# imatge-upc/rsis

Hardware: AMD Instinct MI355X
Metric: training images/sec at 256x256, T=10, batch=32 per GPU (higher is better)
Workload: dtype f32

## Files before the change

rsis_amd/csrc/api.hip:

```cpp
#include "common.h"
#include "../../include/rsis_hip.h"
#include "launchers.h"
#include <stdlib.h>

static inline int krows_of(int C, int ks) { return rsis_roundup(C * ks * ks, RSIS_KPAD); }
static inline int log2i(int s) { int l = 0; while ((1 << l) < s) ++l; return l; }
static inline bool use_direct(int ks, int stride, int pad) { return ks == 3 && stride == 1 && pad == 1; }
static inline bool use_direct_s2(int ks, int stride, int pad) { return ks == 3 && stride == 2 && pad == 1; }
static inline bool use_direct_f2(int ks, int stride, int pad) {
  static const bool on = !(getenv("RSIS_CONV_F2") && getenv("RSIS_CONV_F2")[0] == '0');
  return on && use_direct_s2(ks, stride, pad);
}
static inline bool use_direct_fwd(int ks, int stride, int pad) { return use_direct(ks, stride, pad) || use_direct_f2(ks, stride, pad); }
static inline int seg_chunks(int nseg, const int* Cseg, int ck) {
  int q = 0;
  for (int s = 0; s < nseg; ++s) q += (Cseg[s] + ck - 1) / ck;
  return q;
}
static inline int direct_rows(int nseg, const int* Cseg) { return seg_chunks(nseg, Cseg, RSIS_CK) * RSIS_CK * 9; }
static inline bool bf16_geom(int ks, int stride, int pad, int Cout) {
  return Cout > 1 && ((ks == 3 && stride == 1 && pad == 1) || (ks == 1 && pad == 0));
}
static inline bool use_bf16(int dtype, int ks, int stride, int pad, int Cout) {
  return dtype == RSIS_DTYPE_BF16 && bf16_geom(ks, stride, pad, Cout);
// ... 348 lines not shown
    a.Ho = Hy; a.Wo = Wy; a.oH = Hx; a.oW = Wx;
    return rsis_launch_conv3x3_direct(a, 2, direct_variant(tile), (hipStream_t)stream);
  }
  if (ks == 1 && pad == 0 && stride > 1) {
    if (!inplace && zero_dsts(a, (hipStream_t)stream)) return RSIS_ERR_LAUNCH;
    a.Ho = Hy; a.Wo = Wy; a.stride = 1; a.sshift = 0; a.ostride = stride;
    return rsis_launch_conv_igemm(a, ks, false, 0, tile, (hipStream_t)stream);
  }
  return rsis_launch_conv_igemm(a, ks, true, 0, tile, (hipStream_t)stream);
}

static int wgrad_route(WgradArgs& a, int ks, int lstm_hid, int dtype) {
  if (dtype == RSIS_DTYPE_BF16_BLK) {
    a.blk = 1;
    return rsis_wgrad_bf16_supported(a, ks) ? 1 : -1;
  }
  if (use_direct(ks, a.stride, a.pad) && a.Cout == 1 && lstm_hid == 0 && rsis_c1_supported(a.Cs) && a.H == a.Ho && a.W == a.Wo && a.W % 4 == 0)
    return 0;
  if (dtype == RSIS_DTYPE_BF16 && rsis_wgrad_bf16_supported(a, ks)) return 1;
  static const bool tiled_ok = !(getenv("RSIS_WGRAD_TILED") && getenv("RSIS_WGRAD_TILED")[0] == '0');
  if (tiled_ok && rsis_wgrad_tiled_supported(a, ks)) return 2;
  return 3;
}
static int wgrad_fill(WgradArgs& a, const float* dy, const float* x, float* dW, int B, int Cs, int H, int W, int Cout, int Ho, int Wo,
                      int ks, int stride, int pad, int Ctot, int c_off, int lstm_hid) {
  if (!dy || !x || !dW || c_off < 0 || c_off + Cs > Ctot) return RSIS_ERR_ARG;
  a = WgradArgs{};
  a.dy = dy; a.x = x; a.dw = dW; a.B = B; a.Cs = Cs; a.H = H; a.W = W; a.Ho = Ho; a.Wo = Wo; a.Cout = Cout;
  a.stride = stride; a.pad = pad; a.ldo = Ctot * ks * ks; a.n_off = c_off * ks * ks; a.interleave_hid = lstm_hid;
  return RSIS_OK;
// ... 623 lines not shown
```

rsis_amd/csrc/common.h:

```cpp
#pragma once
#include <hip/hip_runtime.h>
#include <stdint.h>

#define RSIS_OK 0
#define RSIS_ERR_ARG 1
#define RSIS_ERR_LAUNCH 2
#define RSIS_ERR_UNSUPPORTED 3

#define RSIS_KPAD 32
#define RSIS_CK 8
#define RSIS_CKB3 16
#define RSIS_CKB1 64
#define RSIS_LDW_ALIGN 128
#define RSIS_MAX_SRC 3

enum PackMode {
  PACK_IGEMM_FWD = 0,
  PACK_IGEMM_DGRAD = 1,
  PACK_DIRECT_FWD = 2,
  PACK_DIRECT_DGRAD = 3,
  PACK_DIRECT_DGRAD_S2 = 4,
  PACK_BF16_FWD = 5,
  PACK_BF16_DGRAD = 6,
  PACK_WINO_FWD = 7,
// ... 129 lines not shown
    }
  }
}

struct WgradArgs {
  const float* dy;
  const float* x;
  float* dw;
  int B, Cs, H, W, Ho, Wo, Cout;
  int stride, pad;
  int ldo, n_off;
  int interleave_hid;
  int chunk;
  int n_co_tiles, n_n_tiles;
  int blk;
};

struct BlkConvJob {
  const void* src[RSIS_MAX_SRC];
  int C[RSIS_MAX_SRC];
  int nsrc;
  int B, H, W;
  const void* wp;
  int ldw;
  int Cout;
  const float* bias;
  const void* addend;
  void* dst[2];
  int Cd[2];
  int ndst;
// ... 27 lines not shown
```

rsis_amd/csrc/conv_wgrad_bf16.hip:

```cpp
#include "common.h"
#include "launchers.h"

typedef __attribute__((address_space(3))) void* lds_vp_t;
typedef __bf16 bf16x8 __attribute__((ext_vector_type(8)));
typedef __bf16 bf16x2 __attribute__((ext_vector_type(2)));
typedef float f32x2 __attribute__((ext_vector_type(2)));
typedef unsigned u32x4 __attribute__((ext_vector_type(4)));
#define RSIS_OOB 0x7FFFFFF0u

struct WgradBf16Args {
  const float* dy;
  const float* x;
  float* dw;
  int B, Cs, H, W, Cout;
  int ldo, n_off;
  short interleave_hid;
  short blk;
  int n_co_tiles, n_n_tiles, n_sp_tiles, tiles_per_split;
};

__device__ __forceinline__ unsigned wg_pack2(float lo, float hi) {
  const f32x2 f = {lo, hi};
  return __builtin_bit_cast(unsigned, __builtin_convertvector(f, bf16x2));
}
// ... 10 lines not shown
      v[0] = a[0]; v[1] = a[1]; v[2] = a[2]; v[3] = a[3]; v[4] = b[0]; v[5] = b[1]; v[6] = b[2]; v[7] = b[3];
    } else {
#pragma unroll
      for (int i = 0; i < 8; ++i) {
        const bool ok = ok_row && (unsigned)(gx + i) < (unsigned)W;
        v[i] = __builtin_bit_cast(float, __builtin_amdgcn_raw_buffer_load_b32(r, ok ? (unsigned)(off_elems + i) * 4u : RSIS_OOB, 0, 0));
      }
    }
  }
  __device__ __forceinline__ u32x4 cell() const {
    u32x4 c;
#pragma unroll
    for (int k = 0; k < 4; ++k) c[k] = wg_pack2(v[2 * k], v[2 * k + 1]);
    return c;
  }
};

template <int BM, int TW, int IN>
__device__ __forceinline__ void wgrad3_bf16_body(const WgradBf16Args& p, const int bx, const int by) {
#if __HIP_DEVICE_COMPILE__
  constexpr int TP = 64, TH = TP / TW, GPR = TW / 8, NG = TP / 8, KSTEPS = NG / 2;
  constexpr int WGM = BM / 32, KSPW = 4 / WGM, NGG = KSTEPS / KSPW;
  constexpr int PH = TH + 2, XG = GPR + 2, PWP = XG * 8;
  constexpr int ARS = (TP + 8) * 2;
  constexpr int CHSB = (PH * PWP * 2 + 31) / 32 * 32 + 16;
  constexpr int A_BYTES = BM * ARS, X_BYTES = 32 * CHSB, ST_BYTES = A_BYTES + X_BYTES;
  constexpr int NTA = BM * NG / 256;
  constexpr int XT = 32 * PH * XG, NTX = (XT + 255) / 256;
  constexpr int RED_BYTES = 4 * 8 * 288 * 4;
  static_assert(WGM * KSPW == 4 && KSTEPS % KSPW == 0 && (BM * NG) % 256 == 0, "config");
  constexpr int LDS_BYTES = 2 * ST_BYTES > RED_BYTES ? 2 * ST_BYTES : RED_BYTES;
  __shared__ __attribute__((aligned(16))) char lds[LDS_BYTES];

  const int tid = threadIdx.x, lane = tid & 63, l31 = lane & 31, hi = lane >> 5;
  const int wave = __builtin_amdgcn_readfirstlane(tid >> 6);
  const int wm = wave % WGM, wk = wave / WGM;
  const int H = p.H, W = p.W, HW = H * W, Cs = p.Cs, Cout = p.Cout;
  const int co_t = bx % p.n_co_tiles, n_t = bx / p.n_co_tiles;
  const int co0 = co_t * BM, ci0 = n_t * 32;
  const int tiles_x = (W + TW - 1) / TW, tiles_y = (H + TH - 1) / TH;
  const int t_begin = by * p.tiles_per_split;
  const int t_end = min(t_begin + p.tiles_per_split, p.n_sp_tiles);
  if (t_begin >= t_end) return;

  int a_off[NTA], a_y[NTA], a_x[NTA], a_lds[NTA];
#pragma unroll
  for (int i = 0; i < NTA; ++i) {
    const int e = tid + i * 256;
    const int row = e / NG, G = e % NG;
    a_y[i] = G / GPR; a_x[i] = (G % GPR) * 8;
    a_off[i] = co0 + row < Cout ? row * HW + a_y[i] * W + a_x[i] : -1;
    a_lds[i] = row * ARS + G * 16;
  }
  int x_off[NTX], x_y[NTX], x_x[NTX], x_lds[NTX];
#pragma unroll
  for (int i = 0; i < NTX; ++i) {
    const int e = tid + i * 256;
    const int cl = e / (PH * XG), rem = e - cl * (PH * XG);
    const int py = rem / XG, xg = rem - py * XG;
    x_y[i] = py - 1; x_x[i] = (xg - 1) * 8;
    x_off[i] = (e < XT && ci0 + cl < Cs) ? cl * HW + x_y[i] * W + x_x[i] : (int)0x40000000;
    x_lds[i] = cl * CHSB + (py * PWP + xg * 8) * 2;
  }

  const int a_base = (wm * 32 + l31) * ARS + hi * 16;
  int bo[NGG];
#pragma unroll
  for (int gg = 0; gg < NGG; ++gg) {
    const int G = 2 * (gg * KSPW + wk) + hi;
    bo[gg] = l31 * CHSB + ((G / GPR) * PWP + (G % GPR) * 8 + 8) * 2;
  }

  f32x16 acc[9];
#pragma unroll
  for (int t = 0; t < 9; ++t)
#pragma unroll
    for (int r = 0; r < 16; ++r) acc[t][r] = 0.f;

  int tb = t_begin / (tiles_x * tiles_y);
  int trem = t_begin - tb * (tiles_x * tiles_y);
  int ty = trem / tiles_x, tx = trem - ty * tiles_x;

  Task8<IN == 1> ra[NTA], rxp[NTX];
#define W3_LOAD()                                                                                                  \
  {                                                                                                                \
    const int y0 = ty * TH, x0 = tx * TW;                                                                          \
    const float* ab = p.dy + ((size_t)tb * Cout + co0) * HW;                                                       \
    const __amdgpu_buffer_rsrc_t ra_ = __builtin_amdgcn_make_buffer_rsrc((void*)ab, 0, (Cout - co0) * HW * 4, 0x00020000); \
    const int tsc = y0 * W + x0;                                                                                   \
    _Pragma("unroll") for (int i = 0; i < NTA; ++i)                                                                \
      ra[i].load(ra_, a_off[i] + tsc, a_off[i] >= 0 && y0 + a_y[i] < H, x0 + a_x[i], W);                           \
    const float* xb = p.x + ((size_t)tb * Cs + ci0) * HW;                                                          \
    const __amdgpu_buffer_rsrc_t rx_ = __builtin_amdgcn_make_buffer_rsrc((void*)xb, 0, (Cs - ci0) * HW * 4, 0x00020000); \
    _Pragma("unroll") for (int i = 0; i < NTX; ++i)                                                                \
      rxp[i].load(rx_, x_off[i] + tsc, x_off[i] < 0x20000000 && (unsigned)(y0 + x_y[i]) < (unsigned)H, x0 + x_x[i], W); \
    if (++tx == tiles_x) { tx = 0; if (++ty == tiles_y) { ty = 0; ++tb; } }                                        \
  }
#define W3_STORE(BUF)                                                                                              \
  {                                                                                                                \
    char* st = lds + (BUF) * ST_BYTES;                                                                             \
    _Pragma("unroll") for (int i = 0; i < NTA; ++i) *(u32x4*)(st + a_lds[i]) = ra[i].cell();                       \
    _Pragma("unroll") for (int i = 0; i < NTX; ++i)                                                                \
      if (XT % 256 == 0 || tid + i * 256 < XT) *(u32x4*)(st + A_BYTES + x_lds[i]) = rxp[i].cell();                 \
  }

  W3_LOAD() W3_STORE(0)
  __syncthreads();
  const int ntl = t_end - t_begin;
  for (int t = 0; t < ntl; ++t) {
    const int cur = t & 1;
    if (t + 1 < ntl) W3_LOAD()
    {
      const char* As = lds + cur * ST_BYTES + a_base;
      const char* Xs = lds + cur * ST_BYTES + A_BYTES;
#pragma unroll
      for (int gg = 0; gg < NGG; ++gg) {
        const bf16x8 a = __builtin_bit_cast(bf16x8, *(const u32x4*)(As + (gg * KSPW + wk) * 32));
#pragma unroll
        for (int r = 0; r < 3; ++r) {
          const char* row = Xs + bo[gg] + r * PWP * 2;
          const unsigned d0 = *(const unsigned*)(row - 4);
          const u32x4 m = *(const u32x4*)row;
          const unsigned d5 = *(const unsigned*)(row + 16);
          const u32x4 w0 = {__builtin_amdgcn_alignbit(m[0], d0, 16), __builtin_amdgcn_alignbit(m[1], m[0], 16),
                            __builtin_amdgcn_alignbit(m[2], m[1], 16), __builtin_amdgcn_alignbit(m[3], m[2], 16)};
          const u32x4 w2 = {__builtin_amdgcn_alignbit(m[1], m[0], 16), __builtin_amdgcn_alignbit(m[2], m[1], 16),
                            __builtin_amdgcn_alignbit(m[3], m[2], 16), __builtin_amdgcn_alignbit(d5, m[3], 16)};
          acc[r * 3 + 0] = __builtin_amdgcn_mfma_f32_32x32x16_bf16(a, __builtin_bit_cast(bf16x8, w0), acc[r * 3 + 0], 0, 0, 0);
          acc[r * 3 + 1] = __builtin_amdgcn_mfma_f32_32x32x16_bf16(a, __builtin_bit_cast(bf16x8, m), acc[r * 3 + 1], 0, 0, 0);
          acc[r * 3 + 2] = __builtin_amdgcn_mfma_f32_32x32x16_bf16(a, __builtin_bit_cast(bf16x8, w2), acc[r * 3 + 2], 0, 0, 0);
        }
      }
    }
    if (t + 1 < ntl) W3_STORE(cur ^ 1)
    __syncthreads();
  }
#undef W3_LOAD
#undef W3_STORE

  float* red = (float*)lds + wm * (8 * 288);
  const int nvalid = min(32, Cs - ci0) * 9;
#pragma unroll
  for (int q = 0; q < 4; ++q) {
#pragma unroll
    for (int k = 0; k < KSPW; ++k) {
      if (wk == k) {
#pragma unroll
        for (int t = 0; t < 9; ++t)
#pragma unroll
          for (int r = 0; r < 4; ++r) {
            float* d = red + (r + 4 * hi) * 288 + l31 * 9 + t;
            if (k == 0) *d = acc[t][4 * q + r];
            else *d += acc[t][4 * q + r];
// ... 356 lines not shown
#ifndef W3T_TH_64_32
#define W3T_TH_64_32 4
#define W3T_NR_64_32 2
#endif
#ifndef W3T_TH_64_16
#define W3T_TH_64_16 8
#define W3T_NR_64_16 2
#endif
constexpr int w3t_th(int bm, int tw) {
  return tw == 32 ? (bm == 128 ? 2 : (bm == 64 ? W3T_TH_64_32 : W3T_TH_32_32)) : (tw == 16 ? (bm == 128 ? 4 : (bm == 64 ? W3T_TH_64_16 : 8)) : 8);
}
constexpr int w3t_nr(int bm, int tw) {
  return tw == 32 ? (bm == 128 ? 2 : (bm == 64 ? W3T_NR_64_32 : W3T_NR_32_32)) : (tw == 16 ? (bm == 32 ? 3 : (bm == 64 ? W3T_NR_64_16 : 2)) : (bm == 128 ? 2 : 3));
}

template <int BM, int BN, int WGM, int WGN, int TW, int IN>
__device__ __forceinline__ void wgrad1_bf16_body(const WgradBf16Args& p, const int bx, const int by) {
#if __HIP_DEVICE_COMPILE__
  constexpr int TP = 64, TH = TP / TW, GPR = TW / 8, NG = TP / 8, KSTEPS = NG / 2;
  constexpr int TM = BM / WGM / 32, TN = BN / WGN / 32;
  constexpr int ARS = (TP + 8) * 2;
  constexpr int A_BYTES = BM * ARS, B_BYTES = BN * ARS, ST_BYTES = A_BYTES + B_BYTES;
  constexpr int NTA = BM * NG / 256, NTB = BN * NG / 256;
  static_assert(WGM * WGN == 4 && (BM * NG) % 256 == 0 && (BN * NG) % 256 == 0, "config");
  __shared__ __attribute__((aligned(16))) char lds[2 * ST_BYTES];

  const int tid = threadIdx.x, lane = tid & 63, l31 = lane & 31, hi = lane >> 5;
  const int wave = __builtin_amdgcn_readfirstlane(tid >> 6);
  const int wm = wave / WGN, wn = wave % WGN;
  const int H = p.H, W = p.W, HW = H * W, Cs = p.Cs, Cout = p.Cout;
  const int co_t = bx % p.n_co_tiles, n_t = bx / p.n_co_tiles;
  const int co0 = co_t * BM, n0 = n_t * BN;
  const int tiles_x = (W + TW - 1) / TW, tiles_y = (H + TH - 1) / TH;
  const int t_begin = by * p.tiles_per_split;
  const int t_end = min(t_begin + p.tiles_per_split, p.n_sp_tiles);
  if (t_begin >= t_end) return;

  int a_off[NTA], a_y[NTA], a_x[NTA], a_lds[NTA];
#pragma unroll
  for (int i = 0; i < NTA; ++i) {
// ... 14 lines not shown
  }
  const int a_base = (wm * TM * 32 + l31) * ARS + hi * 16;
  const int b_base = (wn * TN * 32 + l31) * ARS + hi * 16;

  f32x16 acc[TM][TN];
#pragma unroll
  for (int i = 0; i < TM; ++i)
#pragma unroll
    for (int j = 0; j < TN; ++j)
#pragma unroll
      for (int r = 0; r < 16; ++r) acc[i][j][r] = 0.f;

  int tb = t_begin / (tiles_x * tiles_y);
  int trem = t_begin - tb * (tiles_x * tiles_y);
  int ty = trem / tiles_x, tx = trem - ty * tiles_x;

  Task8<IN == 1> ra[NTA], rb[NTB];
#define W1_LOAD()                                                                                                  \
  {                                                                                                                \
    const int y0 = ty * TH, x0 = tx * TW;                                                                          \
    const int tsc = y0 * W + x0;                                                                                   \
    const float* ab = p.dy + ((size_t)tb * Cout + co0) * HW;                                                       \
    const __amdgpu_buffer_rsrc_t ra_ = __builtin_amdgcn_make_buffer_rsrc((void*)ab, 0, (Cout - co0) * HW * 4, 0x00020000); \
    _Pragma("unroll") for (int i = 0; i < NTA; ++i)                                                                \
      ra[i].load(ra_, a_off[i] + tsc, a_off[i] >= 0 && y0 + a_y[i] < H, x0 + a_x[i], W);                           \
    const float* xb = p.x + ((size_t)tb * Cs + n0) * HW;                                                           \
    const __amdgpu_buffer_rsrc_t rb_ = __builtin_amdgcn_make_buffer_rsrc((void*)xb, 0, (Cs - n0) * HW * 4, 0x00020000); \
    _Pragma("unroll") for (int i = 0; i < NTB; ++i)                                                                \
      rb[i].load(rb_, b_off[i] + tsc, b_off[i] >= 0 && y0 + b_y[i] < H, x0 + b_x[i], W);                           \
    if (++tx == tiles_x) { tx = 0; if (++ty == tiles_y) { ty = 0; ++tb; } }                                        \
  }
#define W1_STORE(BUF)                                                                                              \
  {                                                                                                                \
    char* st = lds + (BUF) * ST_BYTES;                                                                             \
    _Pragma("unroll") for (int i = 0; i < NTA; ++i) *(u32x4*)(st + a_lds[i]) = ra[i].cell();                       \
    _Pragma("unroll") for (int i = 0; i < NTB; ++i) *(u32x4*)(st + A_BYTES + b_lds[i]) = rb[i].cell();             \
  }

  W1_LOAD() W1_STORE(0)
  __syncthreads();
  const int ntl = t_end - t_begin;
  for (int t = 0; t < ntl; ++t) {
    const int cur = t & 1;
    if (t + 1 < ntl) W1_LOAD()
    {
      const char* As = lds + cur * ST_BYTES + a_base;
      const char* Bs = lds + cur * ST_BYTES + A_BYTES + b_base;
#pragma unroll
      for (int g = 0; g < KSTEPS; ++g) {
        bf16x8 a[TM], b[TN];
#pragma unroll
        for (int i = 0; i < TM; ++i) a[i] = __builtin_bit_cast(bf16x8, *(const u32x4*)(As + i * 32 * ARS + g * 32));
#pragma unroll
        for (int j = 0; j < TN; ++j) b[j] = __builtin_bit_cast(bf16x8, *(const u32x4*)(Bs + j * 32 * ARS + g * 32));
#pragma unroll
        for (int i = 0; i < TM; ++i)
#pragma unroll
          for (int j = 0; j < TN; ++j) acc[i][j] = __builtin_amdgcn_mfma_f32_32x32x16_bf16(a[i], b[j], acc[i][j], 0, 0, 0);
      }
    }
    if (t + 1 < ntl) W1_STORE(cur ^ 1)
    __syncthreads();
  }
#undef W1_LOAD
#undef W1_STORE

  const __amdgpu_buffer_rsrc_t rdw = __builtin_amdgcn_make_buffer_rsrc((void*)p.dw, 0, (unsigned)((size_t)Cout * p.ldo * 4), 0x00020000);
  const int ihid = p.interleave_hid;
  const unsigned ldb = (unsigned)p.ldo * 4u;
#pragma unroll
  for (int j = 0; j < TN; ++j) {
    const int n = n0 + wn * TN * 32 + j * 32 + l31;
    if (n >= Cs) continue;
#pragma unroll
    for (int i = 0; i < TM; ++i) {
      const int row0 = co0 + wm * TM * 32 + i * 32 + 4 * hi;
      const int rows_left = Cout - row0;
      const unsigned vo = (unsigned)((ihid > 0 ? row0 >> 2 : row0) * p.ldo + p.n_off + n) * 4u;
#pragma unroll
      for (int r = 0; r < 16; ++r) {
// ... 61 lines not shown
  wgrad1_tr_body<BM, BN, TP, NR>(g.job[j], tile, split);
}
template <int BM, int BN, int TP, int NR>
static void w1t_launch_group(const WgradBf16Group& g, int blocks, hipStream_t st) {
  constexpr int lds = w1t_lds_bytes<BM, BN, TP, NR>();
  static const hipError_t once = hipFuncSetAttribute((const void*)wgrad1_tr_group_kernel<BM, BN, TP, NR>, hipFuncAttributeMaxDynamicSharedMemorySize, lds);
  (void)once;
  hipLaunchKernelGGL((wgrad1_tr_group_kernel<BM, BN, TP, NR>), dim3(blocks), dim3(256), lds, st, g);
}
template <int BM, int BN, int WGM, int WGN, int TW, int IN>
__global__ __launch_bounds__(256) void wgrad1_bf16_group_kernel(const WgradBf16Group g) {
  int j, tile, split;
  if (!wgb_find(g, j, tile, split)) return;
  wgrad1_bf16_body<BM, BN, WGM, WGN, TW, IN>(g.job[j], tile, split);
}

static void split_plan(WgradBf16Args& a, int TW, int TH, int ntile, int slots) {
  a.n_sp_tiles = a.B * rsis_cdiv(a.H, TH) * rsis_cdiv(a.W, TW);
  int nsplit = ntile >= slots ? 1 : slots / ntile;
  if (nsplit > 256) nsplit = 256;
  if (nsplit > a.n_sp_tiles / 2) nsplit = a.n_sp_tiles / 2;
  if (nsplit < 1 || rsis_deterministic()) nsplit = 1;
  a.tiles_per_split = rsis_cdiv(a.n_sp_tiles, nsplit);
}

bool rsis_wgrad_bf16_supported(const WgradArgs& w, int ks) {
  if (!(ks == 1 || ks == 3) || w.stride != 1 || w.pad != ks / 2 || w.H != w.Ho || w.W != w.Wo) return false;
  if (w.Cout == 1) return false;
  if (w.blk && ((w.Cout & 7) || (w.Cs & 7))) return false;
  const long img = (long)w.H * w.W * 4;
  return (long)w.Cout * img < (1L << 30) && (long)w.Cs * img < (1L << 30);
}

struct WgbKey { int ks, bm, bn, tw, v4, th; };
static WgbKey wgb_key(const WgradBf16Args& a, int ks) {
  WgbKey k = {ks, 0, 0, 0, 0, 0};
  if (ks == 3) {
    k.tw = a.W > 16 ? 32 : (a.W > 8 ? 16 : 8);
    k.bm = a.Cout <= 32 ? 32 : ((a.Cout <= 64 || a.Cs <= 512) ? 64 : 128);
    k.bn = 32;
  } else {
    k.tw = a.blk ? W1T_TP : 64;
    k.bm = a.Cout <= 64 ? 64 : 128;
    k.bn = a.Cs <= 64 ? 64 : 128;
  }
  k.v4 = a.blk ? 2 : (a.W % 4 == 0 ? 1 : 0);
  k.th = ks == 3 ? (a.blk ? w3t_th(k.bm, k.tw) : 64 / k.tw) : (a.blk ? 1 : 64 / k.tw);
  return k;
}
static inline bool wgb_same(const WgbKey& a, const WgbKey& b) { return a.ks == b.ks && a.bm == b.bm && a.bn == b.bn && a.tw == b.tw && a.v4 == b.v4; }

template <typename LaunchFn>
static int wgb_launch_bucket(WgradBf16Args* jobs, int n, const WgbKey& k, bool alone, LaunchFn launch) {
  const int TH = k.th;
  long total = 0;
  for (int j = 0; j < n; ++j) {
    WgradBf16Args& a = jobs[j];
    a.n_co_tiles = rsis_cdiv(a.Cout, k.bm);
    a.n_n_tiles = rsis_cdiv(a.Cs, k.bn);
    a.n_sp_tiles = a.B * rsis_cdiv(a.H, TH) * rsis_cdiv(a.W, k.tw);
    total += (long)a.n_co_tiles * a.n_n_tiles * a.n_sp_tiles;
  }
  if (alone) {
    WgradBf16Group g = {};
    const int ntile = jobs[0].n_co_tiles * jobs[0].n_n_tiles;
// ... 47 lines not shown
      g.lane_split0[best][e] = (unsigned short)items[i].split;
      blocks[best] += items[i].blocks;
      load[best] += items[i].work;
    }
    int maxb = 0;
    for (int x = 0; x < 8; ++x) { g.lane_start[x][g.lane_n[x]] = blocks[x]; if (blocks[x] > maxb) maxb = blocks[x]; }
    launch(g, 8 * maxb);
    if (rsis_check_launch() != RSIS_OK) return RSIS_ERR_LAUNCH;
    j0 += nj;
  }
  return RSIS_OK;
}

#define WGB3(BMv, TWv)                                                                                             \
  if (k.bm == BMv && k.tw == TWv) {                                                                                \
    if (k.v4 == 2) return wgb_launch_bucket(jobs, n, k, alone, [&](const WgradBf16Group& g, int blocks) {                 \
      w3t_launch_group<BMv, TWv, w3t_th(BMv, TWv), w3t_nr(BMv, TWv)>(g, blocks, st); });                           \
    if (k.v4 == 1) return wgb_launch_bucket(jobs, n, k, alone, [&](const WgradBf16Group& g, int blocks) {                 \
      hipLaunchKernelGGL((wgrad3_bf16_group_kernel<BMv, TWv, 1>), dim3(blocks), dim3(256), 0, st, g); });          \
    return wgb_launch_bucket(jobs, n, k, alone, [&](const WgradBf16Group& g, int blocks) {                                \
      hipLaunchKernelGGL((wgrad3_bf16_group_kernel<BMv, TWv, 0>), dim3(blocks), dim3(256), 0, st, g); });          \
  }
#define WGB1(BMv, BNv)                                                                                             \
  if (k.bm == BMv && k.bn == BNv) {                                                                                \
    if (k.v4 == 2) return wgb_launch_bucket(jobs, n, k, alone, [&](const WgradBf16Group& g, int blocks) {                 \
      w1t_launch_group<BMv, BNv, W1T_TP, w1t_nr(BMv, BNv)>(g, blocks, st); });                                     \
    if (k.v4 == 1) return wgb_launch_bucket(jobs, n, k, alone, [&](const WgradBf16Group& g, int blocks) {                 \
      hipLaunchKernelGGL((wgrad1_bf16_group_kernel<BMv, BNv, 2, 2, 64, 1>), dim3(blocks), dim3(256), 0, st, g); });      \
    return wgb_launch_bucket(jobs, n, k, alone, [&](const WgradBf16Group& g, int blocks) {                                \
      hipLaunchKernelGGL((wgrad1_bf16_group_kernel<BMv, BNv, 2, 2, 64, 0>), dim3(blocks), dim3(256), 0, st, g); });      \
  }
static int wgb_dispatch(WgradBf16Args* jobs, int n, const WgbKey& k, bool alone, hipStream_t st) {
  if (k.ks == 3) {
    WGB3(32, 32) WGB3(64, 32) WGB3(128, 32) WGB3(32, 16) WGB3(64, 16) WGB3(128, 16) WGB3(32, 8) WGB3(64, 8) WGB3(128, 8)
  } else {
    WGB1(64, 64) WGB1(64, 128) WGB1(128, 64) WGB1(128, 128)
  }
  return RSIS_ERR_ARG;
}
#undef WGB3
#undef WGB1

static int wgb_launch_jobs(const WgradArgs* w, int n, int ks, bool alone, hipStream_t st) {
  if (n < 1) return RSIS_OK;
  WgradBf16Args* all = (WgradBf16Args*)malloc(sizeof(WgradBf16Args) * n * 2);
  WgbKey* key = (WgbKey*)malloc(sizeof(WgbKey) * n);
  if (!all || !key) { free(all); free(key); return RSIS_ERR_LAUNCH; }
  WgradBf16Args* bucket = all + n;
  for (int j = 0; j < n; ++j) {
    WgradBf16Args a = {};
    a.dy = w[j].dy; a.x = w[j].x; a.dw = w[j].dw; a.B = w[j].B; a.Cs = w[j].Cs; a.H = w[j].H; a.W = w[j].W; a.Cout = w[j].Cout;
    a.ldo = w[j].ldo; a.n_off = w[j].n_off; a.interleave_hid = (short)w[j].interleave_hid; a.blk = (short)w[j].blk;
    if (ks == 1) { a.W = w[j].H * w[j].W; a.H = 1; }
    all[j] = a;
    key[j] = wgb_key(a, ks);
  }
  int rc = RSIS_OK;
  for (int j = 0; j < n && rc == RSIS_OK; ++j) {
    if (key[j].ks < 0) continue;
    const WgbKey k = key[j];
    int m = 0;
    for (int i = j; i < n; ++i)
      if (key[i].ks >= 0 && wgb_same(key[i], k)) { bucket[m++] = all[i]; key[i].ks = -1; }
    rc = wgb_dispatch(bucket, m, k, alone, st);
  }
  free(all); free(key);
  return rc;
}

int rsis_launch_conv_wgrad_bf16_group(const WgradArgs* w, int n, int ks, hipStream_t st) { return wgb_launch_jobs(w, n, ks, false, st); }
// ... 2 lines not shown
```

rsis_amd/csrc/launchers.h:

```cpp
#pragma once
#include "common.h"
#include "../../include/rsis_hip.h"

int rsis_launch_conv_igemm(ConvArgs& a, int ks, bool dgrad, int epi, int force_tile, hipStream_t st);
int rsis_launch_conv3x3_direct(ConvArgs& a, int epi, int force_variant, hipStream_t st);
int rsis_launch_convlstm_direct_group(ConvArgs* jobs, int n, const int* force_variant, hipStream_t st);
int rsis_launch_conv3x3_direct_group_plain(ConvArgs* jobs, int n, const int* force_variant, hipStream_t st);
int rsis_launch_conv_wino(const float* x, const void* U, const float* bias, const float* addend, float* y, int B, int C, int Cout, int H, int W, hipStream_t st,
                          int precise);
int rsis_launch_conv_wino_group(int n, const float* const* x, const void* const* U, float* const* y, float* const* y1, const int* B, const int* C, const int* Cout,
                                const int* C0, const int* H, const int* W, hipStream_t st);
int rsis_launch_conv_bf16(ConvArgs& a, int ks, int epi, int force_variant, hipStream_t st);
int rsis_launch_conv_blk(ConvArgs& a, int ks, int variant, hipStream_t st);
int rsis_l_blk_from_nchw(const float* x, void* y, int B, int C, int HW, hipStream_t st);
int rsis_l_blk_to_nchw(const void* x, float* y, int B, int C, int HW, hipStream_t st);
int rsis_launch_conv_blk_dec(BlkConvJob* jobs, int n, int epi, const int* force_variant, hipStream_t st);
int rsis_launch_conv_wgrad(WgradArgs& a, int ks, hipStream_t st);
bool rsis_wgrad_bf16_supported(const WgradArgs& w, int ks);
int rsis_launch_conv_wgrad_bf16_group(const WgradArgs* w, int n, int ks, hipStream_t st);
int rsis_launch_conv_wgrad_bf16(const WgradArgs& w, int ks, hipStream_t st);
int rsis_launch_conv_wgrad_tiled_group(const WgradArgs* w, int n, int ks, hipStream_t st);
int rsis_launch_conv_wgrad_tiled(const WgradArgs& w, int ks, hipStream_t st);
bool rsis_wgrad_tiled_supported(const WgradArgs& w, int ks);
bool rsis_c1_supported(int Cin);
int rsis_l_c1_fwd(const float* x, const float* wp, int ldw, const float* bias, float* y, int B, int Cin, int H, int W, int seqT, hipStream_t st);
int rsis_l_c1_dgrad(const float* dy, const float* wd, int ldw, float* dx, int B, int Cin, int H, int W, int seqT, hipStream_t st);
int rsis_l_c1_wgrad(const float* dy, const float* x, float* dw, float* db, int B, int Cin, int H, int W, int seqT, hipStream_t st);
bool rsis_upconv_supported(int C, int Hs, int Ws, int Ho, int Wo);
int rsis_upconv_bwd_blocks(int T, int B, int Hs, int Ws);
int rsis_l_upconv_fwd(const void* h, int h_blk, const float* w, const float* bias, float* out, int T, int B, int Hs, int Ws, int Ho, int Wo, hipStream_t st);
int rsis_l_upconv_bwd(const float* dout, const void* h, int h_blk, const float* w, void* dh, float* dW, float* db, const float* dside, const int* arg,
                      float* partial, int T, int B, int Hs, int Ws, int Ho, int Wo, hipStream_t st);
int rsis_l_pack_batch(const rsis_pack_job* jobs, int njobs, int total_blocks, hipStream_t st);
// ... 88 lines not shown
```

rsis_amd/csrc/limb_split.h:

```cpp
#pragma once

#if defined(__HIPCC__) || defined(__CUDACC__)
#define RSIS_LIMB_HD __host__ __device__
#else
#define RSIS_LIMB_HD
#endif

RSIS_LIMB_HD inline float rsis_limb_hi16(const float v) {
  unsigned u;
  __builtin_memcpy(&u, &v, 4);
  u &= 0xFFFF0000u;
  float r;
  __builtin_memcpy(&r, &u, 4);
  return r;
}

RSIS_LIMB_HD inline void rsis_limb_split3(const float v, float& l0, float& l1, float& l2) {
  l0 = rsis_limb_hi16(v);
  const float r1 = v - l0;
  l1 = rsis_limb_hi16(r1);
  l2 = r1 - l1;
}
```

Before: 963.8.

## Route f32 weight-gradient convs through bf16 MFMA with three-limb split

Adds a path that splits each f32 operand into three bf16 limbs while staging into LDS and computes the weight gradient with six bf16 MFMA products per step, approximating f32 accuracy on matrix cores. By default it is enabled only for selected 3x3 shape classes (tile width 32, in both the small-Cout and large-Cout groups) when not in deterministic mode, and env vars can force it on for all supported shapes or turn it off. The limb kernels use dynamic LDS sized for three planes with a single buffer, so they lose the double-buffered overlap. The large-tile variant also keeps a second set of accumulators that it flushes after every tile, which adds register pressure.

```diff
diff --git a/rsis_amd/csrc/api.hip b/rsis_amd/csrc/api.hip
--- a/rsis_amd/csrc/api.hip
+++ b/rsis_amd/csrc/api.hip
@@ -386,6 +386,11 @@
   if (dtype == RSIS_DTYPE_BF16_BLK) {
     a.blk = 1;
     return rsis_wgrad_bf16_supported(a, ks) ? 1 : -1;
+  }
+  if (dtype != RSIS_DTYPE_BF16) {
+    const int staged = rsis_wgrad_staged_limbs(a, ks);
+    if (staged < 0) return -1;
+    if (staged > 0) { a.limbs = 1; return 1; }
   }
   if (use_direct(ks, a.stride, a.pad) && a.Cout == 1 && lstm_hid == 0 && rsis_c1_supported(a.Cs) && a.H == a.Ho && a.W == a.Wo && a.W % 4 == 0)
     return 0;
diff --git a/rsis_amd/csrc/common.h b/rsis_amd/csrc/common.h
--- a/rsis_amd/csrc/common.h
+++ b/rsis_amd/csrc/common.h
@@ -167,6 +167,7 @@
   int chunk;
   int n_co_tiles, n_n_tiles;
   int blk;
+  int limbs;
 };
 
 struct BlkConvJob {
diff --git a/rsis_amd/csrc/conv_wgrad_bf16.hip b/rsis_amd/csrc/conv_wgrad_bf16.hip
--- a/rsis_amd/csrc/conv_wgrad_bf16.hip
+++ b/rsis_amd/csrc/conv_wgrad_bf16.hip
@@ -1,5 +1,8 @@
 #include "common.h"
 #include "launchers.h"
+#include "limb_split.h"
+#include <stdlib.h>
+#include <string.h>
 
 typedef __attribute__((address_space(3))) void* lds_vp_t;
 typedef __bf16 bf16x8 __attribute__((ext_vector_type(8)));
@@ -48,12 +51,31 @@
     for (int k = 0; k < 4; ++k) c[k] = wg_pack2(v[2 * k], v[2 * k + 1]);
     return c;
   }
+  __device__ __forceinline__ void limb_cells(u32x4 (&c)[3]) const {
+    unsigned q[3][4];
+    rsis_limb_pack8_cells(v, q[0], q[1], q[2]);
+#pragma unroll
+    for (int l = 0; l < 3; ++l) c[l] = u32x4{q[l][0], q[l][1], q[l][2], q[l][3]};
+  }
 };
 
-template <int BM, int TW, int IN>
+template <int BYTES, bool DYN>
+__device__ __forceinline__ char* wgb_stage_lds() {
+  if constexpr (DYN) {
+    extern __shared__ __attribute__((aligned(1024))) char wgb_dyn_lds[];
+    return wgb_dyn_lds;
+  } else {
+    __shared__ __attribute__((aligned(16))) char wgb_static_lds[BYTES];
+    return wgb_static_lds;
+  }
+}
+
+template <int BM, int TW, int IN, int LIMBS = 0>
 __device__ __forceinline__ void wgrad3_bf16_body(const WgradBf16Args& p, const int bx, const int by) {
 #if __HIP_DEVICE_COMPILE__
   constexpr int TP = 64, TH = TP / TW, GPR = TW / 8, NG = TP / 8, KSTEPS = NG / 2;
+  constexpr int NPL = LIMBS ? 3 : 1, NBUF = LIMBS ? 1 : 2;
+  constexpr bool FLUSH = LIMBS && BM == 128;
   constexpr int WGM = BM / 32, KSPW = 4 / WGM, NGG = KSTEPS / KSPW;
   constexpr int PH = TH + 2, XG = GPR + 2, PWP = XG * 8;
   constexpr int ARS = (TP + 8) * 2;
@@ -63,8 +85,8 @@
   constexpr int XT = 32 * PH * XG, NTX = (XT + 255) / 256;
   constexpr int RED_BYTES = 4 * 8 * 288 * 4;
   static_assert(WGM * KSPW == 4 && KSTEPS % KSPW == 0 && (BM * NG) % 256 == 0, "config");
-  constexpr int LDS_BYTES = 2 * ST_BYTES > RED_BYTES ? 2 * ST_BYTES : RED_BYTES;
-  __shared__ __attribute__((aligned(16))) char lds[LDS_BYTES];
+  constexpr int LDS_BYTES = NBUF * NPL * ST_BYTES > RED_BYTES ? NBUF * NPL * ST_BYTES : RED_BYTES;
+  char* const lds = wgb_stage_lds<LDS_BYTES, LIMBS != 0>();
 
   const int tid = threadIdx.x, lane = tid & 63, l31 = lane & 31, hi = lane >> 5;
   const int wave = __builtin_amdgcn_readfirstlane(tid >> 6);
@@ -78,24 +100,28 @@
   if (t_begin >= t_end) return;
 
   int a_off[NTA], a_y[NTA], a_x[NTA], a_lds[NTA];
-#pragma unroll
-  for (int i = 0; i < NTA; ++i) {
-    const int e = tid + i * 256;
-    const int row = e / NG, G = e % NG;
-    a_y[i] = G / GPR; a_x[i] = (G % GPR) * 8;
-    a_off[i] = co0 + row < Cout ? row * HW + a_y[i] * W + a_x[i] : -1;
-    a_lds[i] = row * ARS + G * 16;
-  }
   int x_off[NTX], x_y[NTX], x_x[NTX], x_lds[NTX];
-#pragma unroll
-  for (int i = 0; i < NTX; ++i) {
-    const int e = tid + i * 256;
-    const int cl = e / (PH * XG), rem = e - cl * (PH * XG);
-    const int py = rem / XG, xg = rem - py * XG;
-    x_y[i] = py - 1; x_x[i] = (xg - 1) * 8;
-    x_off[i] = (e < XT && ci0 + cl < Cs) ? cl * HW + x_y[i] * W + x_x[i] : (int)0x40000000;
-    x_lds[i] = cl * CHSB + (py * PWP + xg * 8) * 2;
-  }
+#define W3_TASKS(T)                                                                                                \
+  {                                                                                                                \
+    _Pragma("unroll") for (int i = 0; i < NTA; ++i) {                                                              \
+      const int e = (T) + i * 256;                                                                                 \
+      const int row = e / NG, G = e % NG;                                                                          \
+      a_y[i] = G / GPR; a_x[i] = (G % GPR) * 8;                                                                    \
+      a_off[i] = co0 + row < Cout ? row * HW + a_y[i] * W + a_x[i] : -1;                                           \
+      a_lds[i] = row * ARS + G * 16;                                                                               \
+    }                                                                                                              \
+    _Pragma("unroll") for (int i = 0; i < NTX; ++i) {                                                              \
+      const int e = (T) + i * 256;                                                                                 \
+      const int cl = e / (PH * XG), rem = e - cl * (PH * XG);                                                      \
+      const int py = rem / XG, xg = rem - py * XG;                                                                 \
+      x_y[i] = py - 1; x_x[i] = (xg - 1) * 8;                                                                      \
+      x_off[i] = (e < XT && ci0 + cl < Cs) ? cl * HW + x_y[i] * W + x_x[i] : (int)0x40000000;    \
+      x_lds[i] = cl * CHSB + (py * PWP + xg * 8) * 2;                                                              \
+    }                                                                                                              \
+  }
+  constexpr bool RETASK = LIMBS && BM < 128;
+#define W3_RETASK() if constexpr (RETASK) { int tv = tid; asm volatile("" : "+v"(tv)); W3_TASKS(tv) }
+  W3_TASKS(tid)
 
   const int a_base = (wm * 32 + l31) * ARS + hi * 16;
   int bo[NGG];
@@ -110,6 +136,14 @@
   for (int t = 0; t < 9; ++t)
 #pragma unroll
     for (int r = 0; r < 16; ++r) acc[t][r] = 0.f;
+
+  [[maybe_unused]] f32x16 tot[FLUSH ? 9 : 1];
+  if constexpr (FLUSH) {
+#pragma unroll
+    for (int t = 0; t < 9; ++t)
+#pragma unroll
+      for (int r = 0; r < 16; ++r) tot[t][r] = 0.f;
+  }
 
   int tb = t_begin / (tiles_x * tiles_y);
   int trem = t_begin - tb * (tiles_x * tiles_y);
@@ -133,18 +167,69 @@
 #define W3_STORE(BUF)                                                                                              \
   {                                                                                                                \
     char* st = lds + (BUF) * ST_BYTES;                                                                             \
-    _Pragma("unroll") for (int i = 0; i < NTA; ++i) *(u32x4*)(st + a_lds[i]) = ra[i].cell();                       \
-    _Pragma("unroll") for (int i = 0; i < NTX; ++i)                                                                \
-      if (XT % 256 == 0 || tid + i * 256 < XT) *(u32x4*)(st + A_BYTES + x_lds[i]) = rxp[i].cell();                 \
+    if constexpr (LIMBS) {                                                                                         \
+      u32x4 c[3];                                                                                                  \
+      _Pragma("unroll") for (int i = 0; i < NTA; ++i) {                                                            \
+        ra[i].limb_cells(c);                                                                                       \
+        _Pragma("unroll") for (int l = 0; l < 3; ++l) *(u32x4*)(st + l * ST_BYTES + a_lds[i]) = c[l];              \
+      }                                                                                                            \
+      _Pragma("unroll") for (int i = 0; i < NTX; ++i)                                                              \
+        if (XT % 256 == 0 || tid + i * 256 < XT) {                                                                 \
+          rxp[i].limb_cells(c);                                                                                    \
+          _Pragma("unroll") for (int l = 0; l < 3; ++l) *(u32x4*)(st + l * ST_BYTES + A_BYTES + x_lds[i]) = c[l];  \
+        }                                                                                                          \
+    } else {                                                                                                       \
+      _Pragma("unroll") for (int i = 0; i < NTA; ++i) *(u32x4*)(st + a_lds[i]) = ra[i].cell();                     \
+      _Pragma("unroll") for (int i = 0; i < NTX; ++i)                                                              \
+        if (XT % 256 == 0 || tid + i * 256 < XT) *(u32x4*)(st + A_BYTES + x_lds[i]) = rxp[i].cell();               \
+    }                                                                                                              \
   }
 
   W3_LOAD() W3_STORE(0)
   __syncthreads();
   const int ntl = t_end - t_begin;
   for (int t = 0; t < ntl; ++t) {
-    const int cur = t & 1;
-    if (t + 1 < ntl) W3_LOAD()
-    {
+    const int cur = LIMBS ? 0 : t & 1;
+    if (t + 1 < ntl) { W3_RETASK() W3_LOAD() }
+    if constexpr (LIMBS) {
+      const char* As = lds + a_base;
+      const char* Xs = lds + A_BYTES;
+#pragma unroll
+      for (int gg = 0; gg < NGG; ++gg) {
+        bf16x8 a[3];
+#pragma unroll
+        for (int l = 0; l < 3; ++l) a[l] = __builtin_bit_cast(bf16x8, *(const u32x4*)(As + l * ST_BYTES + (gg * KSPW + wk) * 32));
+#pragma unroll
+        for (int r = 0; r < 3; ++r) {
+          bf16x8 w[3][3];
+#pragma unroll
+          for (int l = 0; l < 3; ++l) {
+            const char* row = Xs + l * ST_BYTES + bo[gg] + r * PWP * 2;
+            const unsigned d0 = *(const unsigned*)(row - 4);
+            const u32x4 m = *(const u32x4*)row;
+            const unsigned d5 = *(const unsigned*)(row + 16);
+            const u32x4 w0 = {__builtin_amdgcn_alignbit(m[0], d0, 16), __builtin_amdgcn_alignbit(m[1], m[0], 16),
+                              __builtin_amdgcn_alignbit(m[2], m[1], 16), __builtin_amdgcn_alignbit(m[3], m[2], 16)};
+            const u32x4 w2 = {__builtin_amdgcn_alignbit(m[1], m[0], 16), __builtin_amdgcn_alignbit(m[2], m[1], 16),
+                              __builtin_amdgcn_alignbit(m[3], m[2], 16), __builtin_amdgcn_alignbit(d5, m[3], 16)};
+            w[l][0] = __builtin_bit_cast(bf16x8, w0); w[l][1] = __builtin_bit_cast(bf16x8, m); w[l][2] = __builtin_bit_cast(bf16x8, w2);
+          }
+#pragma unroll
+          for (int q = 0; q < RSIS_LIMB_PRODUCTS; ++q)
+#pragma unroll
+            for (int s = 0; s < 3; ++s)
+              acc[r * 3 + s] = __builtin_amdgcn_mfma_f32_32x32x16_bf16(a[RSIS_LIMB_PA(q)], w[RSIS_LIMB_PB(q)][s], acc[r * 3 + s], 0, 0, 0);
+          if constexpr (BM < 128 && TW == 32) __builtin_amdgcn_sched_barrier(0);
+        }
+      }
+      __syncthreads();
+      if constexpr (FLUSH) {
+#pragma unroll
+        for (int tt = 0; tt < 9; ++tt)
+#pragma unroll
+          for (int r = 0; r < 16; ++r) { tot[tt][r] += acc[tt][r]; acc[tt][r] = 0.f; }
+      }
+    } else {
       const char* As = lds + cur * ST_BYTES + a_base;
       const char* Xs = lds + cur * ST_BYTES + A_BYTES;
 #pragma unroll
@@ -166,11 +251,17 @@
         }
       }
     }
-    if (t + 1 < ntl) W3_STORE(cur ^ 1)
+    if (t + 1 < ntl) { W3_RETASK() W3_STORE(LIMBS ? 0 : cur ^ 1) }
     __syncthreads();
   }
 #undef W3_LOAD
 #undef W3_STORE
+#undef W3_TASKS
+#undef W3_RETASK
+  if constexpr (FLUSH) {
+#pragma unroll
+    for (int t = 0; t < 9; ++t) acc[t] = tot[t];
+  }
 
   float* red = (float*)lds + wm * (8 * 288);
   const int nvalid = min(32, Cs - ci0) * 9;
@@ -557,16 +648,17 @@
   return tw == 32 ? (bm == 128 ? 2 : (bm == 64 ? W3T_NR_64_32 : W3T_NR_32_32)) : (tw == 16 ? (bm == 32 ? 3 : (bm == 64 ? W3T_NR_64_16 : 2)) : (bm == 128 ? 2 : 3));
 }
 
-template <int BM, int BN, int WGM, int WGN, int TW, int IN>
+template <int BM, int BN, int WGM, int WGN, int TW, int IN, int LIMBS = 0>
 __device__ __forceinline__ void wgrad1_bf16_body(const WgradBf16Args& p, const int bx, const int by) {
 #if __HIP_DEVICE_COMPILE__
   constexpr int TP = 64, TH = TP / TW, GPR = TW / 8, NG = TP / 8, KSTEPS = NG / 2;
+  constexpr int NPL = LIMBS ? 3 : 1, NBUF = LIMBS ? 1 : 2;
   constexpr int TM = BM / WGM / 32, TN = BN / WGN / 32;
   constexpr int ARS = (TP + 8) * 2;
   constexpr int A_BYTES = BM * ARS, B_BYTES = BN * ARS, ST_BYTES = A_BYTES + B_BYTES;
   constexpr int NTA = BM * NG / 256, NTB = BN * NG / 256;
   static_assert(WGM * WGN == 4 && (BM * NG) % 256 == 0 && (BN * NG) % 256 == 0, "config");
-  __shared__ __attribute__((aligned(16))) char lds[2 * ST_BYTES];
+  char* const lds = wgb_stage_lds<NBUF * NPL * ST_BYTES, LIMBS != 0>();
 
   const int tid = threadIdx.x, lane = tid & 63, l31 = lane & 31, hi = lane >> 5;
   const int wave = __builtin_amdgcn_readfirstlane(tid >> 6);
@@ -611,6 +703,16 @@
   int tb = t_begin / (tiles_x * tiles_y);
   int trem = t_begin - tb * (tiles_x * tiles_y);
   int ty = trem / tiles_x, tx = trem - ty * tiles_x;
+
+  [[maybe_unused]] f32x16 tot[LIMBS ? TM : 1][LIMBS ? TN : 1];
+  if constexpr (LIMBS) {
+#pragma unroll
+    for (int i = 0; i < TM; ++i)
+#pragma unroll
+      for (int j = 0; j < TN; ++j)
+#pragma unroll
+        for (int r = 0; r < 16; ++r) tot[i][j][r] = 0.f;
+  }
 
   Task8<IN == 1> ra[NTA], rb[NTB];
 #define W1_LOAD()                                                                                                  \
@@ -630,17 +732,57 @@
 #define W1_STORE(BUF)                                                                                              \
   {                                                                                                                \
     char* st = lds + (BUF) * ST_BYTES;                                                                             \
-    _Pragma("unroll") for (int i = 0; i < NTA; ++i) *(u32x4*)(st + a_lds[i]) = ra[i].cell();                       \
-    _Pragma("unroll") for (int i = 0; i < NTB; ++i) *(u32x4*)(st + A_BYTES + b_lds[i]) = rb[i].cell();             \
+    if constexpr (LIMBS) {                                                                                         \
+      u32x4 c[3];                                                                                                  \
+      _Pragma("unroll") for (int i = 0; i < NTA; ++i) {                                                            \
+        ra[i].limb_cells(c);                                                                                       \
+        _Pragma("unroll") for (int l = 0; l < 3; ++l) *(u32x4*)(st + l * ST_BYTES + a_lds[i]) = c[l];              \
+      }                                                                                                            \
+      _Pragma("unroll") for (int i = 0; i < NTB; ++i) {                                                            \
+        rb[i].limb_cells(c);                                                                                       \
+        _Pragma("unroll") for (int l = 0; l < 3; ++l) *(u32x4*)(st + l * ST_BYTES + A_BYTES + b_lds[i]) = c[l];    \
+      }                                                                                                            \
+    } else {                                                                                                       \
+      _Pragma("unroll") for (int i = 0; i < NTA; ++i) *(u32x4*)(st + a_lds[i]) = ra[i].cell();                     \
+      _Pragma("unroll") for (int i = 0; i < NTB; ++i) *(u32x4*)(st + A_BYTES + b_lds[i]) = rb[i].cell();           \
+    }                                                                                                              \
   }
 
   W1_LOAD() W1_STORE(0)
   __syncthreads();
   const int ntl = t_end - t_begin;
   for (int t = 0; t < ntl; ++t) {
-    const int cur = t & 1;
+    const int cur = LIMBS ? 0 : t & 1;
     if (t + 1 < ntl) W1_LOAD()
-    {
+    if constexpr (LIMBS) {
+      const char* As = lds + a_base;
+      const char* Bs = lds + A_BYTES + b_base;
+#pragma unroll
+      for (int g = 0; g < KSTEPS; ++g) {
+        bf16x8 a[TM][3], b[TN][3];
+#pragma unroll
+        for (int l = 0; l < 3; ++l) {
+#pragma unroll
+          for (int i = 0; i < TM; ++i) a[i][l] = __builtin_bit_cast(bf16x8, *(const u32x4*)(As + l * ST_BYTES + i * 32 * ARS + g * 32));
+#pragma unroll
+          for (int j = 0; j < TN; ++j) b[j][l] = __builtin_bit_cast(bf16x8, *(const u32x4*)(Bs + l * ST_BYTES + j * 32 * ARS + g * 32));
+        }
+#pragma unroll
+        for (int q = 0; q < RSIS_LIMB_PRODUCTS; ++q)
+#pragma unroll
+          for (int i = 0; i < TM; ++i)
+#pragma unroll
+            for (int j = 0; j < TN; ++j)
+              acc[i][j] = __builtin_amdgcn_mfma_f32_32x32x16_bf16(a[i][RSIS_LIMB_PA(q)], b[j][RSIS_LIMB_PB(q)], acc[i][j], 0, 0, 0);
+      }
+      __syncthreads();
+#pragma unroll
+      for (int i = 0; i < TM; ++i)
+#pragma unroll
+        for (int j = 0; j < TN; ++j)
+#pragma unroll
+          for (int r = 0; r < 16; ++r) { tot[i][j][r] += acc[i][j][r]; acc[i][j][r] = 0.f; }
+    } else {
       const char* As = lds + cur * ST_BYTES + a_base;
       const char* Bs = lds + cur * ST_BYTES + A_BYTES + b_base;
 #pragma unroll
@@ -656,11 +798,17 @@
           for (int j = 0; j < TN; ++j) acc[i][j] = __builtin_amdgcn_mfma_f32_32x32x16_bf16(a[i], b[j], acc[i][j], 0, 0, 0);
       }
     }
-    if (t + 1 < ntl) W1_STORE(cur ^ 1)
+    if (t + 1 < ntl) W1_STORE(LIMBS ? 0 : cur ^ 1)
     __syncthreads();
   }
 #undef W1_LOAD
 #undef W1_STORE
+  if constexpr (LIMBS) {
+#pragma unroll
+    for (int i = 0; i < TM; ++i)
+#pragma unroll
+      for (int j = 0; j < TN; ++j) acc[i][j] = tot[i][j];
+  }
 
   const __amdgpu_buffer_rsrc_t rdw = __builtin_amdgcn_make_buffer_rsrc((void*)p.dw, 0, (unsigned)((size_t)Cout * p.ldo * 4), 0x00020000);
   const int ihid = p.interleave_hid;
@@ -752,6 +900,42 @@
   if (!wgb_find(g, j, tile, split)) return;
   wgrad1_bf16_body<BM, BN, WGM, WGN, TW, IN>(g.job[j], tile, split);
 }
+template <int BM, int TW>
+constexpr int w3l_lds_bytes() {
+  constexpr int PH = 64 / TW + 2, PWP = (TW / 8 + 2) * 8, CHSB = (PH * PWP * 2 + 31) / 32 * 32 + 16;
+  constexpr int st = 3 * (BM * (64 + 8) * 2 + 32 * CHSB);
+  return st > 4 * 8 * 288 * 4 ? st : 4 * 8 * 288 * 4;
+}
+template <int BM, int BN>
+constexpr int w1l_lds_bytes() { return 3 * (BM + BN) * (64 + 8) * 2; }
+template <int BM, int TW, int IN>
+__global__ __launch_bounds__(256, BM == 128 ? 1 : 2) void wgrad3_limb_group_kernel(const WgradBf16Group g) {
+  int j, tile, split;
+  if (!wgb_find(g, j, tile, split)) return;
+  wgrad3_bf16_body<BM, TW, IN, 1>(g.job[j], tile, split);
+}
+template <int BM, int BN, int IN>
+__global__ __launch_bounds__(256) void wgrad1_limb_group_kernel(const WgradBf16Group g) {
+  int j, tile, split;
+  if (!wgb_find(g, j, tile, split)) return;
+  wgrad1_bf16_body<BM, BN, 2, 2, 64, IN, 1>(g.job[j], tile, split);
+}
+template <int BM, int TW, int IN>
+static void w3l_launch_group(const WgradBf16Group& g, int blocks, hipStream_t st) {
+  constexpr int lds = w3l_lds_bytes<BM, TW>();
+  static_assert(lds <= 160 * 1024, "LDS of a CU");
+  static const hipError_t once = hipFuncSetAttribute((const void*)wgrad3_limb_group_kernel<BM, TW, IN>, hipFuncAttributeMaxDynamicSharedMemorySize, lds);
+  (void)once;
+  hipLaunchKernelGGL((wgrad3_limb_group_kernel<BM, TW, IN>), dim3(blocks), dim3(256), lds, st, g);
+}
+template <int BM, int BN, int IN>
+static void w1l_launch_group(const WgradBf16Group& g, int blocks, hipStream_t st) {
+  constexpr int lds = w1l_lds_bytes<BM, BN>();
+  static_assert(lds <= 160 * 1024, "LDS of a CU");
+  static const hipError_t once = hipFuncSetAttribute((const void*)wgrad1_limb_group_kernel<BM, BN, IN>, hipFuncAttributeMaxDynamicSharedMemorySize, lds);
+  (void)once;
+  hipLaunchKernelGGL((wgrad1_limb_group_kernel<BM, BN, IN>), dim3(blocks), dim3(256), lds, st, g);
+}
 
 static void split_plan(WgradBf16Args& a, int TW, int TH, int ntile, int slots) {
   a.n_sp_tiles = a.B * rsis_cdiv(a.H, TH) * rsis_cdiv(a.W, TW);
@@ -770,9 +954,31 @@
   return (long)w.Cout * img < (1L << 30) && (long)w.Cs * img < (1L << 30);
 }
 
-struct WgbKey { int ks, bm, bn, tw, v4, th; };
-static WgbKey wgb_key(const WgradBf16Args& a, int ks) {
-  WgbKey k = {ks, 0, 0, 0, 0, 0};
+static int wgl_class(const WgradArgs& w, int ks) {
+  if (ks == 3) {
+    const int twi = w.W > 16 ? 2 : (w.W > 8 ? 1 : 0), tw = 8 << twi;
+    if (w.Cs % 32 || w.W % tw || w.H % (64 / tw)) return -1;
+    return (w.Cout > 64 ? 0 : 3) + twi;
+  }
+  if ((w.H * w.W) % 64 || w.Cout <= 32) return -1;
+  return w.Cout >= 128 && w.Cs >= 128 ? 6 : 7;
+}
+static unsigned wgl_class_mask() { return 1u << 5 | 1u << 2; }
+int rsis_wgrad_staged_limbs(const WgradArgs& w, int ks) {
+  static const int mode = [] {
+    const char* e = getenv("RSIS_WGRAD_LIMBS");
+    if (!e || !e[0]) return 0;
+    return strcmp(e, "staged") == 0 ? 2 : 1;
+  }();
+  if (mode == 2) return rsis_wgrad_bf16_supported(w, ks) ? 1 : -1;
+  if (mode == 1 || rsis_deterministic() || !rsis_wgrad_bf16_supported(w, ks)) return 0;
+  const int cls = wgl_class(w, ks);
+  return cls >= 0 && ((wgl_class_mask() >> cls) & 1u);
+}
+
+struct WgbKey { int ks, bm, bn, tw, v4, th, limbs; };
+static WgbKey wgb_key(const WgradBf16Args& a, int ks, int limbs) {
+  WgbKey k = {ks, 0, 0, 0, 0, 0, a.blk ? 0 : limbs};
   if (ks == 3) {
     k.tw = a.W > 16 ? 32 : (a.W > 8 ? 16 : 8);
     k.bm = a.Cout <= 32 ? 32 : ((a.Cout <= 64 || a.Cs <= 512) ? 64 : 128);
@@ -786,7 +992,7 @@
   k.th = ks == 3 ? (a.blk ? w3t_th(k.bm, k.tw) : 64 / k.tw) : (a.blk ? 1 : 64 / k.tw);
   return k;
 }
-static inline bool wgb_same(const WgbKey& a, const WgbKey& b) { return a.ks == b.ks && a.bm == b.bm && a.bn == b.bn && a.tw == b.tw && a.v4 == b.v4; }
+static inline bool wgb_same(const WgbKey& a, const WgbKey& b) { return a.ks == b.ks && a.bm == b.bm && a.bn == b.bn && a.tw == b.tw && a.v4 == b.v4 && a.limbs == b.limbs; }
 
 template <typename LaunchFn>
 static int wgb_launch_bucket(WgradBf16Args* jobs, int n, const WgbKey& k, bool alone, LaunchFn launch) {
@@ -864,6 +1070,10 @@
 
 #define WGB3(BMv, TWv)                                                                                             \
   if (k.bm == BMv && k.tw == TWv) {                                                                                \
+    if (k.limbs && k.v4 == 1) return wgb_launch_bucket(jobs, n, k, alone, [&](const WgradBf16Group& g, int blocks) {      \
+      w3l_launch_group<BMv, TWv, 1>(g, blocks, st); });                                                            \
+    if (k.limbs) return wgb_launch_bucket(jobs, n, k, alone, [&](const WgradBf16Group& g, int blocks) {                   \
+      w3l_launch_group<BMv, TWv, 0>(g, blocks, st); });                                                            \
     if (k.v4 == 2) return wgb_launch_bucket(jobs, n, k, alone, [&](const WgradBf16Group& g, int blocks) {                 \
       w3t_launch_group<BMv, TWv, w3t_th(BMv, TWv), w3t_nr(BMv, TWv)>(g, blocks, st); });                           \
     if (k.v4 == 1) return wgb_launch_bucket(jobs, n, k, alone, [&](const WgradBf16Group& g, int blocks) {                 \
@@ -873,6 +1083,10 @@
   }
 #define WGB1(BMv, BNv)                                                                                             \
   if (k.bm == BMv && k.bn == BNv) {                                                                                \
+    if (k.limbs && k.v4 == 1) return wgb_launch_bucket(jobs, n, k, alone, [&](const WgradBf16Group& g, int blocks) {      \
+      w1l_launch_group<BMv, BNv, 1>(g, blocks, st); });                                                            \
+    if (k.limbs) return wgb_launch_bucket(jobs, n, k, alone, [&](const WgradBf16Group& g, int blocks) {                   \
+      w1l_launch_group<BMv, BNv, 0>(g, blocks, st); });                                                            \
     if (k.v4 == 2) return wgb_launch_bucket(jobs, n, k, alone, [&](const WgradBf16Group& g, int blocks) {                 \
       w1t_launch_group<BMv, BNv, W1T_TP, w1t_nr(BMv, BNv)>(g, blocks, st); });                                     \
     if (k.v4 == 1) return wgb_launch_bucket(jobs, n, k, alone, [&](const WgradBf16Group& g, int blocks) {                 \
@@ -903,7 +1117,7 @@
     a.ldo = w[j].ldo; a.n_off = w[j].n_off; a.interleave_hid = (short)w[j].interleave_hid; a.blk = (short)w[j].blk;
     if (ks == 1) { a.W = w[j].H * w[j].W; a.H = 1; }
     all[j] = a;
-    key[j] = wgb_key(a, ks);
+    key[j] = wgb_key(a, ks, w[j].limbs);
   }
   int rc = RSIS_OK;
   for (int j = 0; j < n && rc == RSIS_OK; ++j) {
diff --git a/rsis_amd/csrc/launchers.h b/rsis_amd/csrc/launchers.h
--- a/rsis_amd/csrc/launchers.h
+++ b/rsis_amd/csrc/launchers.h
@@ -17,6 +17,7 @@
 int rsis_launch_conv_blk_dec(BlkConvJob* jobs, int n, int epi, const int* force_variant, hipStream_t st);
 int rsis_launch_conv_wgrad(WgradArgs& a, int ks, hipStream_t st);
 bool rsis_wgrad_bf16_supported(const WgradArgs& w, int ks);
+int rsis_wgrad_staged_limbs(const WgradArgs& w, int ks);
 int rsis_launch_conv_wgrad_bf16_group(const WgradArgs* w, int n, int ks, hipStream_t st);
 int rsis_launch_conv_wgrad_bf16(const WgradArgs& w, int ks, hipStream_t st);
 int rsis_launch_conv_wgrad_tiled_group(const WgradArgs* w, int n, int ks, hipStream_t st);
diff --git a/rsis_amd/csrc/limb_split.h b/rsis_amd/csrc/limb_split.h
--- a/rsis_amd/csrc/limb_split.h
+++ b/rsis_amd/csrc/limb_split.h
@@ -21,3 +21,25 @@
   l1 = rsis_limb_hi16(r1);
   l2 = r1 - l1;
 }
+
+RSIS_LIMB_HD inline unsigned rsis_limb_pair(const float even, const float odd) {
+  unsigned e, o;
+  __builtin_memcpy(&e, &even, 4);
+  __builtin_memcpy(&o, &odd, 4);
+  return (e >> 16) | (o & 0xFFFF0000u);
+}
+
+RSIS_LIMB_HD inline void rsis_limb_pack8_cells(const float (&v)[8], unsigned (&c0)[4], unsigned (&c1)[4], unsigned (&c2)[4]) {
+  for (int m = 0; m < 4; ++m) {
+    float lo[3], hi[3];
+    rsis_limb_split3(v[2 * m], lo[0], lo[1], lo[2]);
+    rsis_limb_split3(v[2 * m + 1], hi[0], hi[1], hi[2]);
+    c0[m] = rsis_limb_pair(v[2 * m], v[2 * m + 1]);
+    c1[m] = rsis_limb_pair(lo[1], hi[1]);
+    c2[m] = rsis_limb_pair(lo[2], hi[2]);
+  }
+}
+
+#define RSIS_LIMB_PRODUCTS 6
+#define RSIS_LIMB_PA(q) ((q) == 1 ? 2 : ((q) == 2 || (q) == 4 ? 1 : 0))
+#define RSIS_LIMB_PB(q) ((q) == 0 ? 2 : ((q) == 2 || (q) == 3 ? 1 : 0))
```

After: 973.7, median of 6. +1.0%, better.
